# retir/Style-Big-GAN

Hardware: AMD Instinct MI355X
Metric: images/sec (G+D step) StyleGAN2-ADA 256x256 bf16 (higher is better)
Workload: dtype bf16; 1 GPU; configs/sg2ada.yaml @ 256x256: sg2_classic G (skip) + D (orig), softplus + R1(0.01)/4, idle Greg slot /16 (G lr x 16/17), global batch 64 = 1 rank(s) x 2 round(s) x batch_gpu 32 (the rounds of a phase evaluated in one pass, minibatch-std groups and loss those of the separate rounds), bf16 from 8x8 up (num_fp16_res 6; the reference recipe defaults to 4), conv_clamp 256, ADA off; global_batch=64, per_rank_batch=64, parallelism=dp1

## Files before the change

include/sbg_hip.h:

```cpp
#ifndef SBG_HIP_H
#define SBG_HIP_H

#include <stdint.h>

#ifdef __cplusplus
extern "C" {
#endif

typedef void* sbg_stream_t;

enum sbg_status {
    SBG_OK = 0,
    SBG_ERR_INVALID = 1,
    SBG_ERR_UNSUPPORTED = 2,
    SBG_ERR_LAUNCH = 3
};

enum sbg_dtype { SBG_F32 = 0, SBG_F16 = 1, SBG_BF16 = 2 };

enum sbg_act {
    SBG_ACT_LINEAR = 1, SBG_ACT_RELU = 2, SBG_ACT_LRELU = 3, SBG_ACT_TANH = 4, SBG_ACT_SIGMOID = 5,
    SBG_ACT_ELU = 6, SBG_ACT_SELU = 7, SBG_ACT_SOFTPLUS = 8, SBG_ACT_SWISH = 9
};

// ... 44 lines not shown
    int accumulate;
    const float* bias; const float* noise; int64_t noise_stride_n;
    int act; float alpha, gain, clamp;
    void* workspace; int ksplit;
    int nphase; int ph_ntaps[4], ph_oh[4], ph_ow[4]; int64_t ph_yoff[4];
} sbg_conv_params;
int64_t sbg_conv2d_igemm_workspace(const sbg_conv_params* p);
int     sbg_conv2d_igemm(const sbg_conv_params* p, sbg_stream_t stream);


typedef struct sbg_wgrad_params {
    const void* a; const void* b; float* out; void* workspace;
    int dtype;
    int N, PH, PW, Ca, BH, BW, Cb;
    int64_t as_n, as_h, as_w;
    int64_t bs_n, bs_h, bs_w;
    int stride;
    int ntaps;
    int tap_dy[SBG_MAX_TAPS], tap_dx[SBG_MAX_TAPS];
    int accumulate;
} sbg_wgrad_params;
int64_t sbg_conv2d_wgrad_workspace(const sbg_wgrad_params* p);
int     sbg_conv2d_wgrad(const sbg_wgrad_params* p, sbg_stream_t stream);


int sbg_scale_nc(const void* x, const float* a, const float* z, void* y, int dtype, int layout,
                 int N, int C, int64_t HW, int64_t z_stride_n, sbg_stream_t stream);
int sbg_scale_shift_nc(const void* x, const float* a, const float* b, void* y, int dtype, int layout,
                       int N, int C, int64_t HW, sbg_stream_t stream);

int sbg_dot_hw_splits(int layout, int N, int C, int64_t HW);
int sbg_dot_hw(const void* u, const void* v, float* partial, int dtype, int layout,
               int N, int C, int64_t HW, sbg_stream_t stream);
int sbg_moments_hw(const void* x, float* r, int dtype, int N, int C, int64_t HW, sbg_stream_t stream);

typedef struct sbg_gg_problem {
    const float *a0, *b0, *a1, *b1;
    float* c; const float* bias; float* rowsum;
    int64_t a0_rs, a0_cs, b0_rs, b0_cs, a1_rs, a1_cs, b1_rs, b1_cs, c_rs, c_cs;
    int M, N, K0, K1, nterms;
    float alpha0, alpha1, bias_scale, rowsum_scale;
} sbg_gg_problem;
int sbg_grouped_gemm(const sbg_gg_problem* problems, int count, sbg_stream_t stream);

int sbg_dot_hw_scale_supported(int C);
int sbg_dot_hw_scale(const void* u, const void* v, const float* scale, void* y, float* partial, int dtype,
// ... 129 lines not shown
```

style-big-gan_amd/_lib.py:

```python
import ctypes
import os
import threading

import torch

_HERE = os.path.dirname(os.path.abspath(__file__))
LIB_PATH = os.environ.get("SBG_HIP_LIBRARY") or os.path.join(_HERE, "libsbg_hip.so")

SBG_F32, SBG_F16, SBG_BF16 = 0, 1, 2
SBG_MAX_TAPS = 16

_DTYPES = {torch.float32: SBG_F32, torch.float16: SBG_F16, torch.bfloat16: SBG_BF16}


def dtype_code(dtype):
    try:
        return _DTYPES[dtype]
    except KeyError:
        raise RuntimeError(f"style_big_gan_amd: unsupported dtype {dtype} (float32 / float16 / bfloat16 only)")


class UpfirdnParams(ctypes.Structure):
    _fields_ = [
        ("x", ctypes.c_void_p), ("f", ctypes.c_void_p), ("y", ctypes.c_void_p),
# ... 81 lines not shown
QUANT_RULES = {"grid": 0, "clamp": 1}
RESAMPLE_VARIANTS = {0: "h", 1: "v"}
PR_VARIANTS = {0: "single", 1: "split", 2: "merge", 3: "norms"}
ATT_VARIANTS = {0: "single", 1: "stream", 2: "stream_stats", 3: "stream_dq", 4: "stream_dkv"}

_lib = None
_lock = threading.Lock()

_c = ctypes
SYMBOLS = [
    ("sbg_version", _c.c_int, []),
    ("sbg_last_error", _c.c_char_p, []),
    ("sbg_bias_act", _c.c_int, [_c.c_void_p] * 6 + [_c.c_int, _c.c_int, _c.c_int, _c.c_float, _c.c_float, _c.c_float,
                                                   _c.c_int64, _c.c_int, _c.c_int64, _c.c_void_p]),
    ("sbg_upfirdn2d_tail_supported", _c.c_int, [_c.POINTER(UpfirdnParams)]),
    ("sbg_upfirdn2d", _c.c_int, [_c.POINTER(UpfirdnParams), _c.c_void_p]),
    ("sbg_upfirdn2d_dact_rows", _c.c_int64, [_c.POINTER(UpfirdnParams)]),
    ("sbg_upfirdn2d_separable_supported", _c.c_int, [_c.c_int] * 3),
    ("sbg_upfirdn2d_separable", _c.c_int, [_c.c_void_p] * 3 + [_c.c_int] * 11 + [_c.c_float, _c.c_void_p]),
    ("sbg_conv2d_igemm_workspace", _c.c_int64, [_c.POINTER(ConvParams)]),
    ("sbg_conv2d_igemm", _c.c_int, [_c.POINTER(ConvParams), _c.c_void_p]),
    ("sbg_conv2d_wgrad_workspace", _c.c_int64, [_c.POINTER(WgradParams)]),
    ("sbg_conv2d_wgrad", _c.c_int, [_c.POINTER(WgradParams), _c.c_void_p]),
    ("sbg_scale_nc", _c.c_int, [_c.c_void_p] * 4 + [_c.c_int, _c.c_int, _c.c_int, _c.c_int, _c.c_int64, _c.c_int64, _c.c_void_p]),
    ("sbg_scale_shift_nc", _c.c_int, [_c.c_void_p] * 4 + [_c.c_int, _c.c_int, _c.c_int, _c.c_int, _c.c_int64, _c.c_void_p]),
    ("sbg_sn_workspace", _c.c_int64, [_c.c_int, _c.c_int]),
    ("sbg_sn_power_iteration", _c.c_int, [_c.c_void_p] * 6 + [_c.c_int, _c.c_int, _c.c_float, _c.c_void_p]),
    ("sbg_mbstd_workspace", _c.c_int64, [_c.c_int] * 5),
    ("sbg_mbstd_fwd", _c.c_int, [_c.c_void_p] * 3 + [_c.c_int] * 5 + [_c.c_void_p]),
    ("sbg_mbstd_bwd", _c.c_int, [_c.c_void_p] * 3 + [_c.c_int] * 5 + [_c.c_void_p]),
    ("sbg_split_bf16_cat", _c.c_int, [_c.c_void_p, _c.c_void_p, _c.c_int64, _c.c_int64, _c.c_int64, _c.c_int, _c.POINTER(_c.c_int), _c.c_void_p]),
    ("sbg_split_bf16_cat_nd", _c.c_int, [_c.c_void_p, _c.POINTER(_c.c_int64), _c.POINTER(_c.c_int64), _c.c_int, _c.c_void_p, _c.c_int, _c.POINTER(_c.c_int), _c.c_void_p]),
    ("sbg_attention_supported", _c.c_int, [_c.c_int] * 4),
    ("sbg_attention_fwd", _c.c_int, [_c.c_void_p] * 4 + [_c.c_int] * 5 + [_c.c_void_p]),
    ("sbg_attention_bwd_supported", _c.c_int, [_c.c_int] * 4),
    ("sbg_attention_bwd_workspace", _c.c_int64, [_c.c_int, _c.c_int]),
    ("sbg_attention_bwd", _c.c_int, [_c.c_void_p] * 8 + [_c.c_int] * 5 + [_c.c_void_p]),
    ("sbg_dot_hw_splits", _c.c_int, [_c.c_int, _c.c_int, _c.c_int, _c.c_int64]),
    ("sbg_dot_hw", _c.c_int, [_c.c_void_p] * 3 + [_c.c_int, _c.c_int, _c.c_int, _c.c_int, _c.c_int64, _c.c_void_p]),
    ("sbg_moments_hw", _c.c_int, [_c.c_void_p, _c.c_void_p, _c.c_int, _c.c_int, _c.c_int, _c.c_int64, _c.c_void_p]),
    ("sbg_grouped_gemm", _c.c_int, [_c.c_void_p, _c.c_int, _c.c_void_p]),
    ("sbg_dot_hw_scale_supported", _c.c_int, [_c.c_int]),
    ("sbg_dot_hw_scale", _c.c_int, [_c.c_void_p] * 5 + [_c.c_int, _c.c_int, _c.c_int, _c.c_int64, _c.c_void_p]),
    ("sbg_modconv_bwd_supported", _c.c_int, [_c.c_int]),
    ("sbg_modconv_bwd", _c.c_int, [_c.c_void_p] * 8 + [_c.c_int, _c.c_int, _c.c_int, _c.c_int64, _c.c_int64, _c.c_int, _c.c_float, _c.c_float, _c.c_float, _c.c_void_p]),
    ("sbg_modconv_bwd_prescaled", _c.c_int, [_c.c_void_p] * 10 + [_c.c_int, _c.c_int, _c.c_int, _c.c_int64, _c.c_int64, _c.c_int, _c.c_float, _c.c_float, _c.c_float, _c.c_void_p]),
# ... 111 lines not shown
```

style-big-gan_amd/csrc/conv_wgrad.hip:

```cpp
#include "conv_common.h"
#include "lds_asm.h"

namespace {

struct bf16_mfma {}; struct f16_mfma {};
template <class MF> struct Mfma;
template <> struct Mfma<bf16_mfma> {
    static __device__ __forceinline__ float4_t run(short8_t a, short8_t b, float4_t c) {
        return __builtin_amdgcn_mfma_f32_16x16x32_bf16(__builtin_bit_cast(bf16x8_t, a), __builtin_bit_cast(bf16x8_t, b), c, 0, 0, 0);
    }
};
template <> struct Mfma<f16_mfma> {
    static __device__ __forceinline__ float4_t run(short8_t a, short8_t b, float4_t c) {
        return __builtin_amdgcn_mfma_f32_16x16x32_f16(__builtin_bit_cast(f16x8_t, a), __builtin_bit_cast(f16x8_t, b), c, 0, 0, 0);
    }
};

struct WgradArgs {
    const unsigned short* a; const unsigned short* b; float* out; float* ws;
    int N, PH, PW, Ca, BH, BW, Cb;
    int64_t as_n, as_h, as_w, bs_n, bs_h, bs_w;
    int stride, ntaps;
    int tap_dy[SBG_MAX_TAPS], tap_dx[SBG_MAX_TAPS];
    int accumulate;
// ... 146 lines not shown
        float* slab = dst_base + (int64_t)(p.tap0 + t) * p.Ca * p.Cb;
#pragma unroll
        for (int i = 0; i < TA; i++)
#pragma unroll
            for (int j = 0; j < TB; j++) {
                const int cb = cb0 + wb + 16 * j + fi;
                if (cb >= p.Cb) continue;
#pragma unroll
                for (int e = 0; e < 4; e++) {
                    const int ca = ca0 + wa + 16 * i + 4 * fg + e;
                    if (ca >= p.Ca) continue;
                    float* d = slab + (int64_t)ca * p.Cb + cb;
                    const float v = acc[t][i][j][e];
                    *d = (direct && p.accumulate) ? *d + v : v;
                }
            }
    }
}



using sbgconv::lds_void_ptr;

template <class MF, int S, int BCA, int NSTAGE>
__global__ __launch_bounds__(512) void conv_wgrad_rows_kernel(WgradArgs p, unsigned a_bytes, unsigned b_bytes)
{
    static_assert(BCA == 64 || BCA == 128, "a tile of 64 or 128 channels");
    static_assert(NSTAGE >= 2 && NSTAGE <= 6, "2..6 stages (the wait ladder covers five chunks in flight)");
    constexpr int BCB = 64, NT = 9, DEPTH = NSTAGE - 1;
    constexpr int TA = BCA / 32;
    constexpr int APIECES = BCA / 16;
    constexpr int PCOLS = S * 31 + 3;
    constexpr int PPR = (PCOLS + 7) / 8;
    constexpr int PROW = PPR * 8;
    constexpr int NWAVE = 8;
    constexpr int NPIECE = ((APIECES + 3 * PPR + NWAVE - 1) / NWAVE) * NWAVE;
    constexpr int PIECES = NPIECE / NWAVE;
    constexpr int NREAL = APIECES + 3 * PPR;
    constexpr int A_BYTES = APIECES * 1024, STAGE = NREAL * 1024, DUMP = NSTAGE * STAGE;

    extern __shared__ __attribute__((aligned(16))) unsigned char smem[];
    const int tid = threadIdx.x, lane = tid & 63;
    const int wave = __builtin_amdgcn_readfirstlane(tid >> 6);
    int ta_, tb_, split;
    if (!wgrad_decode_block(p, ta_, tb_, split)) return;
    const int ca0 = ta_ * BCA, cb0 = tb_ * BCB;
    const int chunk_begin = split * p.chunks_per_split;
    int chunk_end = chunk_begin + p.chunks_per_split;
    if (chunk_end > p.nchunks) chunk_end = p.nchunks;
    const int nloc = chunk_end - chunk_begin;
    const int xblocks = p.PW >> 5;
    const int dy0 = p.tap_dy[0], dx0 = p.tap_dx[0];

    __amdgpu_buffer_rsrc_t ar = __builtin_amdgcn_make_buffer_rsrc((void*)p.a, 0, (int)a_bytes, 0x00020000);
    __amdgpu_buffer_rsrc_t br = __builtin_amdgcn_make_buffer_rsrc((void*)p.b, 0, (int)b_bytes, 0x00020000);

    const int drow = lane >> 3, dchunk = lane & 7;
    auto src_chunk = [&](int R) { return (((dchunk >> 1) ^ ((R >> 1) & 3)) << 1) | (dchunk & 1); };

    struct ChunkC { int py, n, px0; unsigned char* st; };
    auto chunk_coords = [&](int loc) -> ChunkC {
        const int c = chunk_begin + loc;
        const int xb = c % xblocks, rowid = c / xblocks;
        ChunkC r; r.py = rowid % p.PH; r.n = rowid / p.PH; r.px0 = xb << 5; r.st = smem + (loc % NSTAGE) * STAGE;
        return r;
    };
    auto issue_piece = [&](const ChunkC& cc, int i) {
        const int py = cc.py, n = cc.n, px0 = cc.px0;
        unsigned char* st = cc.st;
        {
            const int piece = wave + NWAVE * i;
            if (piece < APIECES) {
                const int R = (piece & 3) * 8 + drow;
                const int ch = ca0 + (piece >> 2) * 64 + src_chunk(R) * 8;
                const unsigned okm = 0u - (unsigned)(ch < p.Ca);
                const unsigned real = (unsigned)(n * (int)p.as_n + py * (int)p.as_h + (px0 + R) * (int)p.as_w + ch) * 2u;
                __builtin_amdgcn_raw_ptr_buffer_load_lds(ar, (lds_void_ptr)(st + piece * 1024), 16, (real & okm) | (SBG_OOB_OFFSET & ~okm), 0, 0, 0);
            } else {
                const int q = piece - APIECES;
                const int r = q / PPR, jb = q - r * PPR;
                const int R = r * PROW + jb * 8 + drow;
                constexpr int NEVEN = (PCOLS + 1) / 2, EVROWS = ((NEVEN + 7) / 8) * 8;
                const int pcol = (S == 1) ? jb * 8 + drow : (jb * 8 < EVROWS ? 2 * (jb * 8 + drow) : 2 * (jb * 8 - EVROWS + drow) + 1);
                const int by = S * py + dy0 + r, bx = S * px0 + dx0 + pcol;
                const int ch = cb0 + src_chunk(R) * 8;
                const unsigned okm = 0u - (unsigned)((q < 3 * PPR) & (pcol < PCOLS) & ((unsigned)by < (unsigned)p.BH) & ((unsigned)bx < (unsigned)p.BW) & (ch < p.Cb));
                const unsigned real = (unsigned)(n * (int)p.bs_n + by * (int)p.bs_h + bx * (int)p.bs_w + ch) * 2u;
                unsigned char* dst = (q < 3 * PPR) ? st + A_BYTES + q * 1024 : smem + DUMP;
                __builtin_amdgcn_raw_ptr_buffer_load_lds(br, (lds_void_ptr)dst, 16, (real & okm) | (SBG_OOB_OFFSET & ~okm), 0, 0, 0);
            }
        }
    };
    auto issue = [&](int loc) {
        const ChunkC cc = chunk_coords(loc);
#pragma unroll
        for (int i = 0; i < PIECES; i++) issue_piece(cc, i);
    };
    constexpr bool late = true;

    const int wa = (wave >> 2) * (BCA / 2), wb = (wave & 3) * 16;
    const int fi = lane & 15, fg = lane >> 4, fq = fi >> 2, fp = fi & 3;
    const unsigned lds_base = (unsigned)(uintptr_t)((lds_void_ptr)smem);
    float4_t acc[NT][TA];
#pragma unroll
    for (int t = 0; t < NT; t++)
#pragma unroll
        for (int i = 0; i < TA; i++) acc[t][i] = float4_t{0.f, 0.f, 0.f, 0.f};

    auto frag_off = [&](int Rrel, int col) {
        const int chunk = (col >> 3) + (fp >> 1);
        const int sw = (((chunk >> 1) ^ ((Rrel >> 1) & 3)) << 1) | (chunk & 1);
// ... 14 lines not shown
        short4_t lo = lds_tr_read(base + off), hi = lds_tr_read(base + off + hi_off);
        return short8_t{lo[0], lo[1], lo[2], lo[3], hi[0], hi[1], hi[2], hi[3]};
    };

#pragma unroll
    for (int s = 0; s < DEPTH; s++) if (s < nloc) issue(s);
    for (int s = 0; s < nloc; s++) {
        {
            const int later = nloc - 1 - s;
            if (DEPTH >= 2 && later >= DEPTH - 1) asm volatile("s_waitcnt vmcnt(%0)" :: "n"((DEPTH - 1) * PIECES) : "memory");
            else if (DEPTH >= 3 && later == DEPTH - 2) asm volatile("s_waitcnt vmcnt(%0)" :: "n"((DEPTH >= 3 ? DEPTH - 2 : 0) * PIECES) : "memory");
            else if (DEPTH >= 4 && later == DEPTH - 3) asm volatile("s_waitcnt vmcnt(%0)" :: "n"((DEPTH >= 4 ? DEPTH - 3 : 0) * PIECES) : "memory");
            else if (DEPTH >= 5 && later == DEPTH - 4) asm volatile("s_waitcnt vmcnt(%0)" :: "n"((DEPTH >= 5 ? DEPTH - 4 : 0) * PIECES) : "memory");
            else                                       asm volatile("s_waitcnt vmcnt(0)" ::: "memory");
        }
        __builtin_amdgcn_s_barrier();
        const bool more = s + DEPTH < nloc;
        ChunkC nxt = chunk_coords(more ? s + DEPTH : s);
        if (more && !late) {
#pragma unroll
            for (int i = 0; i < PIECES; i++) issue_piece(nxt, i);
        }
        const unsigned stage = lds_base + (unsigned)((s % NSTAGE) * STAGE);
        short4_t alo[TA], ahi[TA], blo[3], bhi[3];
        sbg_static_for<TA>([&](auto it) {
            constexpr int i = decltype(it)::value;
            lds_tr_issue<0>(alo[i], stage + (unsigned)offA[i]);
            lds_tr_issue<16 * 128>(ahi[i], stage + (unsigned)offA[i]);
        });
        unsigned pb[3];
#pragma unroll
        for (int d = 0; d < 3; d++) pb[d] = stage + (unsigned)offB[d];
        auto issue_b = [&](auto tt) {
            constexpr int t = decltype(tt)::value, dyi = t / 3, dxi = t % 3, OFF = A_BYTES + dyi * PROW * 128;
            lds_tr_issue<OFF>(blo[t % 3], pb[dxi]);
            lds_tr_issue<OFF + 16 * 128>(bhi[t % 3], pb[dxi]);
        };
        issue_b(std::integral_constant<int, 0>{});
        issue_b(std::integral_constant<int, 1>{});
        sbg_static_for<9>([&](auto tt) {
            constexpr int t = decltype(tt)::value;
            if constexpr (t + 2 < 9) issue_b(std::integral_constant<int, t + 2>{});
            lds_wait<(t + 2 < 9 ? 4 : t + 1 < 9 ? 2 : 0)>(blo[t % 3], bhi[t % 3]);
            const short8_t fb = short8_t{blo[t % 3][0], blo[t % 3][1], blo[t % 3][2], blo[t % 3][3], bhi[t % 3][0], bhi[t % 3][1], bhi[t % 3][2], bhi[t % 3][3]};
#pragma unroll
            for (int i = 0; i < TA; i++) {
                const short8_t fa_i = short8_t{alo[i][0], alo[i][1], alo[i][2], alo[i][3], ahi[i][0], ahi[i][1], ahi[i][2], ahi[i][3]};
                acc[t][i] = Mfma<MF>::run(fa_i, fb, acc[t][i]);
            }
            if (more && late) {
                sbg_static_for<PIECES>([&](auto pt) {
                    constexpr int i = decltype(pt)::value;
                    if constexpr (i * 9 / PIECES == t) issue_piece(nxt, i);
                });
            }
        });
    }

    const bool direct = (p.nsplit == 1);
    float* dst_base = direct ? p.out : p.ws + (int64_t)split * p.ntaps_total * p.Ca * p.Cb;
    const int cb = cb0 + wb + fi;
#pragma unroll
    for (int t = 0; t < NT; t++) {
        if (t >= p.ntaps || cb >= p.Cb) continue;
        float* slab = dst_base + (int64_t)(p.tap0 + t) * p.Ca * p.Cb;
#pragma unroll
        for (int i = 0; i < TA; i++)
#pragma unroll
            for (int e = 0; e < 4; e++) {
                const int ca = ca0 + wa + 16 * i + 4 * fg + e;
                if (ca >= p.Ca) continue;
                float* d = slab + (int64_t)ca * p.Cb + cb;
                const float v = acc[t][i][e];
                *d = (direct && p.accumulate) ? *d + v : v;
            }
    }
// ... 108 lines not shown
struct ThinPlan { bool ok; int dymin, dxmin, RY, PCOLS, wave_lds, nwg; };

static ThinPlan thin_plan(const sbg_wgrad_params* q)
{
    ThinPlan t; t.ok = false;
    if (q->Ca > 32 || q->Cb > 32 || q->Ca * q->Cb > 512 || q->ntaps > 9 || q->ntaps < 1 || q->stride < 1 || q->stride > 2 || q->N < 1) return t;
    int dy0 = q->tap_dy[0], dy1 = dy0, dx0 = q->tap_dx[0], dx1 = dx0;
    for (int i = 1; i < q->ntaps; i++) {
        if (q->tap_dy[i] < dy0) dy0 = q->tap_dy[i]; if (q->tap_dy[i] > dy1) dy1 = q->tap_dy[i];
        if (q->tap_dx[i] < dx0) dx0 = q->tap_dx[i]; if (q->tap_dx[i] > dx1) dx1 = q->tap_dx[i];
    }
    if (dy1 - dy0 > 2 || dx1 - dx0 > 2) return t;
    t.dymin = dy0; t.dxmin = dx0; t.RY = dy1 - dy0 + 1; t.PCOLS = q->stride * 31 + (dx1 - dx0) + 1;
    t.wave_lds = ((32 * q->Ca + t.RY * t.PCOLS * q->Cb) * 2 + 15) & ~15;
    const int64_t nchunks = (int64_t)q->N * q->PH * ((q->PW + 31) / 32);
    int64_t nwg = (nchunks + 15) / 16;
    if (nwg > 2048) nwg = 2048;
    if (nwg < 1) nwg = 1;
    t.nwg = (int)nwg;
    t.ok = nchunks < INT32_MAX;
    return t;
}

static void plan_split(WgradArgs& a, int bca, int bcb, int target)
{
    a.atiles = (a.Ca + bca - 1) / bca;
    a.btiles = (a.Cb + bcb - 1) / bcb;
    a.nchunks = (int)((a.P + 31) / 32);
    const int tiles = a.atiles * a.btiles;
    int want = (target + tiles - 1) / tiles;
    int maxsplit = a.nchunks / 8; if (maxsplit < 1) maxsplit = 1;
    if (want > maxsplit) want = maxsplit;
    if (want < 1) want = 1;
    a.chunks_per_split = (a.nchunks + want - 1) / want;
    a.nsplit = (a.nchunks + a.chunks_per_split - 1) / a.chunks_per_split;
}

static bool use_big_tile(int ntaps) { return ntaps == 1; }

static int rows_bca(const WgradArgs& a)
{
    return a.Ca >= 128 ? 128 : 64;
}

static constexpr int rows_nstage(int stride, int bca)
{
    if (bca == 128) return 4;
    return stride == 1 ? 4 : 2;
}

static bool rows_kernel_ok(const sbg_wgrad_params* q, const WgradArgs& a)
{
    if ((q->stride != 1 && q->stride != 2) || (q->PW % 32) != 0 || q->ntaps != 9) return false;
    for (int t = 0; t < 9; t++)
        if (q->tap_dy[t] != q->tap_dy[0] + t / 3 || q->tap_dx[t] != q->tap_dx[0] + t % 3) return false;
    if (q->as_n < 0 || q->as_h < 0 || q->as_w < 0 || q->bs_n < 0 || q->bs_h < 0 || q->bs_w < 0) return false;
    const int64_t ab = 2 * ((int64_t)(q->N - 1) * q->as_n + (int64_t)(q->PH - 1) * q->as_h + (int64_t)(q->PW - 1) * q->as_w + q->Ca);
    const int64_t bb = 2 * ((int64_t)(q->N - 1) * q->bs_n + (int64_t)(q->BH - 1) * q->bs_h + (int64_t)(q->BW - 1) * q->bs_w + q->Cb);
    return ab < (int64_t)SBG_OOB_OFFSET && bb < (int64_t)SBG_OOB_OFFSET && a.P > 0;
}

static int fill_args(const sbg_wgrad_params* q, WgradArgs& a)
{
    SBG_CHECK(q && q->a && q->b && q->out, "conv2d_wgrad: null pointer");
    SBG_CHECK(q->dtype == SBG_BF16 || q->dtype == SBG_F16, "conv2d_wgrad: a/b must be bf16 or f16 (fp32 inputs are split by the host)");
    SBG_CHECK(q->N >= 0 && q->PH >= 1 && q->PW >= 1 && q->BH >= 1 && q->BW >= 1, "conv2d_wgrad: bad sizes");
    SBG_CHECK(q->Ca >= 8 && q->Cb >= 8 && (q->Ca % 8) == 0 && (q->Cb % 8) == 0, "conv2d_wgrad: channel counts must be multiples of 8 (pad on the host)");
    SBG_CHECK(q->ntaps >= 1 && q->ntaps <= SBG_MAX_TAPS, "conv2d_wgrad: 1..%d taps", SBG_MAX_TAPS);
    SBG_CHECK(q->stride >= 1, "conv2d_wgrad: stride must be >= 1");
    SBG_CHECK(sbg_aligned16(q->a) && sbg_aligned16(q->b), "conv2d_wgrad: a and b must be 16-byte aligned");
    SBG_CHECK((q->as_n % 8) == 0 && (q->as_h % 8) == 0 && (q->as_w % 8) == 0 && (q->bs_n % 8) == 0 && (q->bs_h % 8) == 0 && (q->bs_w % 8) == 0,
              "conv2d_wgrad: pixel / row strides must be multiples of 8 elements");
    a.a = (const unsigned short*)q->a; a.b = (const unsigned short*)q->b; a.out = q->out; a.ws = (float*)q->workspace;
    a.N = q->N; a.PH = q->PH; a.PW = q->PW; a.Ca = q->Ca; a.BH = q->BH; a.BW = q->BW; a.Cb = q->Cb;
    a.as_n = q->as_n; a.as_h = q->as_h; a.as_w = q->as_w; a.bs_n = q->bs_n; a.bs_h = q->bs_h; a.bs_w = q->bs_w;
    a.stride = q->stride; a.ntaps = q->ntaps; a.accumulate = q->accumulate;
    for (int t = 0; t < SBG_MAX_TAPS; t++) { a.tap_dy[t] = q->tap_dy[t]; a.tap_dx[t] = q->tap_dx[t]; }
    a.P = (int64_t)q->N * q->PH * q->PW;
    a.tap0 = 0; a.ntaps_total = q->ntaps;
    if (use_big_tile(q->ntaps)) plan_split(a, 128, 128, 1024); else plan_split(a, 64, 64, 1024);
    if (rows_kernel_ok(q, a)) plan_split(a, rows_bca(a), 64, 512);
    const ThinPlan tp = thin_plan(q);
    if (tp.ok) { a.atiles = a.btiles = 1; a.nsplit = 4 * tp.nwg; a.chunks_per_split = 0; }
    return SBG_OK;
}

template <class MF, int BCA, int BCB, int NT>
static int launch_wgrad(const WgradArgs& a, hipStream_t stream)
{
    constexpr int lds = 32 * (BCA * 2 + 32) + NT * 32 * (BCB * 2 + 32);
    auto kern = conv_wgrad_kernel<MF, BCA, BCB, NT>;
    if (lds > 64 * 1024 && !SBG_RAISE_LDS_ONCE(kern, lds))
        return sbg_fail(SBG_ERR_LAUNCH, "conv2d_wgrad: cannot raise the dynamic LDS limit to %d bytes", lds);
    SbgProfScope prof(stream, SBG_K_CONV_WGRAD, 2.0 * (double)a.P * a.Ca * (double)a.Cb * a.ntaps,
                      2.0 * (double)a.P * a.Ca + 2.0 * (double)a.N * a.BH * a.BW * a.Cb + 4.0 * a.ntaps * (double)a.Ca * a.Cb * (a.nsplit > 1 ? a.nsplit : 1),
                      {(int)(a.P > INT32_MAX ? INT32_MAX : a.P), a.Ca, a.Cb, a.ntaps, a.stride, a.nsplit, BCA * 1000 + BCB});
    SBG_LAUNCH(kern, dim3(wgrad_grid(a)), dim3(256), lds, stream, a);
    SBG_HIP_LAUNCH_CHECK();
    return SBG_OK;
}

}

extern "C" int64_t sbg_conv2d_wgrad_workspace(const sbg_wgrad_params* q)
{
    WgradArgs a;
    if (fill_args(q, a) != SBG_OK) return -1;
    if (a.nsplit <= 1) return 0;
    return (int64_t)a.nsplit * a.ntaps_total * a.Ca * a.Cb * (int64_t)sizeof(float);
}

extern "C" int sbg_conv2d_wgrad(const sbg_wgrad_params* q, sbg_stream_t stream)
{
    WgradArgs a;
    int rc = fill_args(q, a);
    if (rc != SBG_OK) return rc;
    hipStream_t s = (hipStream_t)stream;
    const int64_t out_n = (int64_t)a.ntaps_total * a.Ca * a.Cb;
    if (a.P == 0) {
        if (!a.accumulate) { if (hipMemsetAsync(a.out, 0, out_n * sizeof(float), s) != hipSuccess) return sbg_fail(SBG_ERR_LAUNCH, "conv2d_wgrad: memset failed"); }
        return SBG_OK;
    }
    SBG_CHECK(a.nsplit == 1 || a.ws != nullptr, "conv2d_wgrad: workspace required (%d pixel splits)", a.nsplit);
    const bool bf = (q->dtype == SBG_BF16);
    const ThinPlan tp = thin_plan(q);
    if (tp.ok) {
        const int ta = (a.Ca + 15) / 16, tb = (a.Cb + 15) / 16;
        const int lds = 4 * tp.wave_lds;
        SbgProfScope prof(s, SBG_K_CONV_WGRAD, 2.0 * (double)a.P * a.Ca * (double)a.Cb * a.ntaps,
                          2.0 * (double)a.P * a.Ca + 2.0 * (double)a.N * a.BH * a.BW * a.Cb + 4.0 * a.ntaps * (double)a.Ca * a.Cb * a.nsplit,
                          {(int)(a.P > INT32_MAX ? INT32_MAX : a.P), a.Ca, a.Cb, a.ntaps, a.stride, a.nsplit, 3000000 + ta * 10 + tb});
#define SBG_THIN_LAUNCH(MFT, A_, B_) do { auto kern = conv_wgrad_thin_kernel<MFT, A_, B_>; \
        if (lds > 64 * 1024 && !SBG_RAISE_LDS_ONCE(kern, lds)) return sbg_fail(SBG_ERR_LAUNCH, "conv2d_wgrad: cannot raise the dynamic LDS limit to %d bytes", lds); \
        SBG_LAUNCH(kern, dim3((unsigned)tp.nwg), dim3(256), lds, s, a, tp.dymin, tp.dxmin, tp.RY, tp.PCOLS, tp.wave_lds); } while (0)
        if (bf) { if (ta == 1 && tb == 1) SBG_THIN_LAUNCH(bf16_mfma, 1, 1); else if (ta == 2 && tb == 1) SBG_THIN_LAUNCH(bf16_mfma, 2, 1);
                  else if (ta == 1) SBG_THIN_LAUNCH(bf16_mfma, 1, 2); else SBG_THIN_LAUNCH(bf16_mfma, 2, 2); }
        else    { if (ta == 1 && tb == 1) SBG_THIN_LAUNCH(f16_mfma, 1, 1); else if (ta == 2 && tb == 1) SBG_THIN_LAUNCH(f16_mfma, 2, 1);
                  else if (ta == 1) SBG_THIN_LAUNCH(f16_mfma, 1, 2); else SBG_THIN_LAUNCH(f16_mfma, 2, 2); }
#undef SBG_THIN_LAUNCH
        SBG_HIP_LAUNCH_CHECK();
    } else if (rows_kernel_ok(q, a)) {
        const unsigned ab = (unsigned)(2 * ((int64_t)(q->N - 1) * q->as_n + (int64_t)(q->PH - 1) * q->as_h + (int64_t)(q->PW - 1) * q->as_w + q->Ca));
        const unsigned bb = (unsigned)(2 * ((int64_t)(q->N - 1) * q->bs_n + (int64_t)(q->BH - 1) * q->bs_h + (int64_t)(q->BW - 1) * q->bs_w + q->Cb));
        const int bca = rows_bca(a);
        const int s_ = q->stride;
        auto stage_kib = [](int S, int BCA) { const int ppr = (S * 31 + 3 + 7) / 8; return BCA / 16 + 3 * ppr; };
        const int lds = (rows_nstage(s_, bca) * stage_kib(s_, bca) + 1) * 1024;
        SbgProfScope prof(s, SBG_K_CONV_WGRAD, 2.0 * (double)a.P * a.Ca * (double)a.Cb * a.ntaps,
                          2.0 * (double)a.P * a.Ca + 2.0 * (double)a.N * a.BH * a.BW * a.Cb + 4.0 * a.ntaps * (double)a.Ca * a.Cb * (a.nsplit > 1 ? a.nsplit : 1),
                          {(int)(a.P > INT32_MAX ? INT32_MAX : a.P), a.Ca, a.Cb, a.ntaps, a.stride, a.nsplit, 1000000 + bca * 1000 + 64});
        const dim3 grid(wgrad_grid(a));
#define SBG_ROWS_LAUNCH(MFT, SS, BB) do { auto kern = conv_wgrad_rows_kernel<MFT, SS, BB, rows_nstage(SS, BB)>; \
        if (lds > 64 * 1024 && !SBG_RAISE_LDS_ONCE(kern, lds)) return sbg_fail(SBG_ERR_LAUNCH, "conv2d_wgrad: cannot raise the dynamic LDS limit to %d bytes", lds); \
        SBG_LAUNCH(kern, grid, dim3(512), lds, s, a, ab, bb); } while (0)
        if (s_ == 1 && bca == 64)       { if (bf) SBG_ROWS_LAUNCH(bf16_mfma, 1, 64);  else SBG_ROWS_LAUNCH(f16_mfma, 1, 64); }
        else if (s_ == 1)               { if (bf) SBG_ROWS_LAUNCH(bf16_mfma, 1, 128); else SBG_ROWS_LAUNCH(f16_mfma, 1, 128); }
        else if (bca == 64)             { if (bf) SBG_ROWS_LAUNCH(bf16_mfma, 2, 64);  else SBG_ROWS_LAUNCH(f16_mfma, 2, 64); }
        else                            { if (bf) SBG_ROWS_LAUNCH(bf16_mfma, 2, 128); else SBG_ROWS_LAUNCH(f16_mfma, 2, 128); }
#undef SBG_ROWS_LAUNCH
        SBG_HIP_LAUNCH_CHECK();
    } else if (use_big_tile(a.ntaps)) {
        rc = bf ? launch_wgrad<bf16_mfma, 128, 128, 1>(a, s) : launch_wgrad<f16_mfma, 128, 128, 1>(a, s);
        if (rc != SBG_OK) return rc;
    } else {
        const int total = a.ntaps;
        for (int t0 = 0; t0 < total; t0 += 9) {
            WgradArgs g = a;
            g.tap0 = t0; g.ntaps = (total - t0 < 9) ? total - t0 : 9;
            for (int t = 0; t < g.ntaps; t++) { g.tap_dy[t] = a.tap_dy[t0 + t]; g.tap_dx[t] = a.tap_dx[t0 + t]; }
            rc = bf ? launch_wgrad<bf16_mfma, 64, 64, 9>(g, s) : launch_wgrad<f16_mfma, 64, 64, 9>(g, s);
            if (rc != SBG_OK) return rc;
        }
    }
    if (a.nsplit > 1) {
        SbgProfScope prof(s, SBG_K_WGRAD_REDUCE, 0.0, 4.0 * out_n * (a.nsplit + 1), {(int)out_n, a.nsplit});
        if (out_n >= (1 << 18) || a.nsplit < 16)
            SBG_LAUNCH(wgrad_reduce_kernel<1>, dim3(sbg_stream_grid(out_n, 256)), dim3(256), 0, s, a.ws, a.out, out_n, a.nsplit, a.accumulate);
        else if (out_n >= (1 << 14))
            SBG_LAUNCH(wgrad_reduce_kernel<4>, dim3(sbg_stream_grid(out_n * 4, 256)), dim3(256), 0, s, a.ws, a.out, out_n, a.nsplit, a.accumulate);
        else
            SBG_LAUNCH(wgrad_reduce_kernel<64>, dim3(sbg_stream_grid(out_n * 64, 256)), dim3(256), 0, s, a.ws, a.out, out_n, a.nsplit, a.accumulate);
// ... 5 lines not shown
```

style-big-gan_amd/torch_utils/ops/conv2d_gradfix.py:

```python
import contextlib

import weakref

import numpy as np

import torch

from ... import _lib

enabled = False
weight_gradients_disabled = False


@contextlib.contextmanager
def no_weight_gradients():
    global weight_gradients_disabled
    old = weight_gradients_disabled
    weight_gradients_disabled = True
    try:
        yield
    finally:
        weight_gradients_disabled = old


# ... 307 lines not shown
                    for j in range(kw) if (b + pw - j) % s == 0]
            if not taps:
                need_zero = True
                continue
            phases.append((a, b, goh, gow, taps))
    multi = len(passes) > 1 or any(len(t) > _lib.SBG_MAX_TAPS for *_, t in phases)
    y = torch.empty([n, cout, oh, ow], dtype=torch.float32 if multi else x.dtype, device=x.device, memory_format=torch.channels_last)
    if need_zero:
        y.zero_()
    first = True
    if (not multi and 2 <= len(phases) <= 4 and sum(len(t) for *_, t in phases) <= _lib.SBG_MAX_TAPS):
        xa, wa = passes[0]
        _igemm_phases(xa, wa.contiguous(), y, phases, s)
        return y
    for xa, wa in passes:
        wa = wa.contiguous()
        for a, b, goh, gow, taps in phases:
            for gi, grp in enumerate(_launch_groups(taps)):
                _igemm(xa, wa, y, grp, 1, goh, gow, y_off=(a, b), y_step=(s, s), accumulate=(not first) or gi > 0)
        first = False
    return y.to(x.dtype) if y.dtype != x.dtype else y


def _wgrad(a, b, stride, taps):
    lib = _lib.load()
    assert a.dtype == b.dtype and a.shape[0] == b.shape[0]
    ca, cb = a.shape[1], b.shape[1]
    pw = a.shape[3]
    if (len(taps) == 9 and stride in (1, 2) and pw in (8, 16)
            and all(taps[t] == (taps[0][0] + t // 3, taps[0][1] + t % 3) for t in range(9))):
        a = torch.nn.functional.pad(a, (0, 32 - pw))
    ap, bp = _pad_channels(a), _pad_channels(b)
    cap, cbp = ap.shape[1], bp.shape[1]
    out = torch.empty([len(taps), cap, cbp], dtype=torch.float32, device=a.device)
    first = True
    for aa, bb in _mfma_operands(ap, bp, 0, 0):
        aa, bb = _cl(aa), _cl(bb)
        for g0 in range(0, len(taps), _lib.SBG_MAX_TAPS):
            grp = taps[g0:g0 + _lib.SBG_MAX_TAPS]
            p = _lib.WgradParams()
            p.a, p.b, p.out = aa.data_ptr(), bb.data_ptr(), out[g0:].data_ptr()
            p.dtype = _lib.dtype_code(aa.dtype)
            p.N, p.PH, p.PW, p.Ca = aa.shape[0], aa.shape[2], aa.shape[3], cap
            p.BH, p.BW, p.Cb = bb.shape[2], bb.shape[3], cbp
            p.as_n, p.as_h, p.as_w = aa.stride(0), aa.stride(2), aa.stride(3)
            p.bs_n, p.bs_h, p.bs_w = bb.stride(0), bb.stride(2), bb.stride(3)
            p.stride, p.ntaps = stride, len(grp)
            for i, (dy, dx) in enumerate(grp):
                p.tap_dy[i], p.tap_dx[i] = dy, dx
            p.accumulate = int(not first)
            nbytes = lib.sbg_conv2d_wgrad_workspace(p)
            if nbytes < 0:
                _lib.check(1, "sbg_conv2d_wgrad_workspace")
            ws = torch.empty([max(nbytes, 4) // 4], dtype=torch.float32, device=a.device) if nbytes > 0 else None
            p.workspace = ws.data_ptr() if ws is not None else None
            _lib.check(lib.sbg_conv2d_wgrad(p, _lib.stream_ptr(a.device)), "sbg_conv2d_wgrad")
        first = False
    return out[:, :ca, :cb]



def _output_padding_for(transpose, stride, padding, in_hw, out_hw, k_hw):
    if transpose:
        return (0, 0)
    return tuple(in_hw[i] - (out_hw[i] - 1) * stride[i] - (1 - 2 * padding[i]) - (k_hw[i] - 1) for i in range(2))


class _Conv(torch.autograd.Function):

    @staticmethod
    def forward(ctx, x, w, cfg):
        transpose, stride, padding, output_padding = cfg[:4]
        wgain = cfg[4] if len(cfg) > 4 else 1.0
# ... 111 lines not shown
```

Baseline: 597.2 img/s.

## Process row pairs per chunk in stride-1 wgrad rows kernel to reuse B rows

Adds an R=2 variant of the rows-based weight-gradient kernel for stride-1, 32-wide inputs. Each chunk now loads two activation rows plus four gradient rows, and every loaded B fragment feeds the MFMAs of both A rows. Each B row used to be loaded for three separate chunks; now it is shared across the pair, cutting LDS staging and global traffic per output row. In exchange, each stage uses more LDS, the 64-channel case drops to two pipeline stages, there are half as many chunks for split-K parallelism, and the Python parameter setup is refactored into a helper.

```diff
diff --git a/include/sbg_hip.h b/include/sbg_hip.h
--- a/include/sbg_hip.h
+++ b/include/sbg_hip.h
@@ -90,6 +90,7 @@
 } sbg_wgrad_params;
 int64_t sbg_conv2d_wgrad_workspace(const sbg_wgrad_params* p);
 int     sbg_conv2d_wgrad(const sbg_wgrad_params* p, sbg_stream_t stream);
+int     sbg_conv2d_wgrad_rows_per_chunk(const sbg_wgrad_params* p);
 
 
 int sbg_scale_nc(const void* x, const float* a, const float* z, void* y, int dtype, int layout,
diff --git a/style-big-gan_amd/_lib.py b/style-big-gan_amd/_lib.py
--- a/style-big-gan_amd/_lib.py
+++ b/style-big-gan_amd/_lib.py
@@ -127,6 +127,7 @@
     ("sbg_conv2d_igemm", _c.c_int, [_c.POINTER(ConvParams), _c.c_void_p]),
     ("sbg_conv2d_wgrad_workspace", _c.c_int64, [_c.POINTER(WgradParams)]),
     ("sbg_conv2d_wgrad", _c.c_int, [_c.POINTER(WgradParams), _c.c_void_p]),
+    ("sbg_conv2d_wgrad_rows_per_chunk", _c.c_int, [_c.POINTER(WgradParams)]),
     ("sbg_scale_nc", _c.c_int, [_c.c_void_p] * 4 + [_c.c_int, _c.c_int, _c.c_int, _c.c_int, _c.c_int64, _c.c_int64, _c.c_void_p]),
     ("sbg_scale_shift_nc", _c.c_int, [_c.c_void_p] * 4 + [_c.c_int, _c.c_int, _c.c_int, _c.c_int, _c.c_int64, _c.c_void_p]),
     ("sbg_sn_workspace", _c.c_int64, [_c.c_int, _c.c_int]),
diff --git a/style-big-gan_amd/csrc/conv_wgrad.hip b/style-big-gan_amd/csrc/conv_wgrad.hip
--- a/style-big-gan_amd/csrc/conv_wgrad.hip
+++ b/style-big-gan_amd/csrc/conv_wgrad.hip
@@ -192,21 +192,24 @@
 
 using sbgconv::lds_void_ptr;
 
-template <class MF, int S, int BCA, int NSTAGE>
+template <class MF, int S, int BCA, int NSTAGE, int R>
 __global__ __launch_bounds__(512) void conv_wgrad_rows_kernel(WgradArgs p, unsigned a_bytes, unsigned b_bytes)
 {
     static_assert(BCA == 64 || BCA == 128, "a tile of 64 or 128 channels");
+    static_assert(R == 1 || R == 2, "one a row or a row pair per chunk");
     static_assert(NSTAGE >= 2 && NSTAGE <= 6, "2..6 stages (the wait ladder covers five chunks in flight)");
     constexpr int BCB = 64, NT = 9, DEPTH = NSTAGE - 1;
     constexpr int TA = BCA / 32;
-    constexpr int APIECES = BCA / 16;
+    constexpr int APT = BCA / 16;
+    constexpr int APIECES = R * APT;
+    constexpr int PR = S * (R - 1) + 3;
     constexpr int PCOLS = S * 31 + 3;
     constexpr int PPR = (PCOLS + 7) / 8;
     constexpr int PROW = PPR * 8;
     constexpr int NWAVE = 8;
-    constexpr int NPIECE = ((APIECES + 3 * PPR + NWAVE - 1) / NWAVE) * NWAVE;
+    constexpr int NPIECE = ((APIECES + PR * PPR + NWAVE - 1) / NWAVE) * NWAVE;
     constexpr int PIECES = NPIECE / NWAVE;
-    constexpr int NREAL = APIECES + 3 * PPR;
+    constexpr int NREAL = APIECES + PR * PPR;
     constexpr int A_BYTES = APIECES * 1024, STAGE = NREAL * 1024, DUMP = NSTAGE * STAGE;
 
     extern __shared__ __attribute__((aligned(16))) unsigned char smem[];
@@ -220,19 +223,20 @@
     if (chunk_end > p.nchunks) chunk_end = p.nchunks;
     const int nloc = chunk_end - chunk_begin;
     const int xblocks = p.PW >> 5;
+    const int prows = (p.PH + R - 1) / R;
     const int dy0 = p.tap_dy[0], dx0 = p.tap_dx[0];
 
     __amdgpu_buffer_rsrc_t ar = __builtin_amdgcn_make_buffer_rsrc((void*)p.a, 0, (int)a_bytes, 0x00020000);
     __amdgpu_buffer_rsrc_t br = __builtin_amdgcn_make_buffer_rsrc((void*)p.b, 0, (int)b_bytes, 0x00020000);
 
     const int drow = lane >> 3, dchunk = lane & 7;
-    auto src_chunk = [&](int R) { return (((dchunk >> 1) ^ ((R >> 1) & 3)) << 1) | (dchunk & 1); };
+    auto src_chunk = [&](int row) { return (((dchunk >> 1) ^ ((row >> 1) & 3)) << 1) | (dchunk & 1); };
 
     struct ChunkC { int py, n, px0; unsigned char* st; };
     auto chunk_coords = [&](int loc) -> ChunkC {
         const int c = chunk_begin + loc;
         const int xb = c % xblocks, rowid = c / xblocks;
-        ChunkC r; r.py = rowid % p.PH; r.n = rowid / p.PH; r.px0 = xb << 5; r.st = smem + (loc % NSTAGE) * STAGE;
+        ChunkC r; r.py = (rowid % prows) * R; r.n = rowid / prows; r.px0 = xb << 5; r.st = smem + (loc % NSTAGE) * STAGE;
         return r;
     };
     auto issue_piece = [&](const ChunkC& cc, int i) {
@@ -241,22 +245,23 @@
         {
             const int piece = wave + NWAVE * i;
             if (piece < APIECES) {
-                const int R = (piece & 3) * 8 + drow;
-                const int ch = ca0 + (piece >> 2) * 64 + src_chunk(R) * 8;
-                const unsigned okm = 0u - (unsigned)(ch < p.Ca);
-                const unsigned real = (unsigned)(n * (int)p.as_n + py * (int)p.as_h + (px0 + R) * (int)p.as_w + ch) * 2u;
+                const int arow = piece / APT, ap = piece % APT;
+                const int R_ = (ap & 3) * 8 + drow;
+                const int ch = ca0 + (ap >> 2) * 64 + src_chunk(R_) * 8;
+                const unsigned okm = 0u - (unsigned)((ch < p.Ca) & (py + arow < p.PH));
+                const unsigned real = (unsigned)(n * (int)p.as_n + (py + arow) * (int)p.as_h + (px0 + R_) * (int)p.as_w + ch) * 2u;
                 __builtin_amdgcn_raw_ptr_buffer_load_lds(ar, (lds_void_ptr)(st + piece * 1024), 16, (real & okm) | (SBG_OOB_OFFSET & ~okm), 0, 0, 0);
             } else {
                 const int q = piece - APIECES;
                 const int r = q / PPR, jb = q - r * PPR;
-                const int R = r * PROW + jb * 8 + drow;
+                const int R_ = r * PROW + jb * 8 + drow;
                 constexpr int NEVEN = (PCOLS + 1) / 2, EVROWS = ((NEVEN + 7) / 8) * 8;
                 const int pcol = (S == 1) ? jb * 8 + drow : (jb * 8 < EVROWS ? 2 * (jb * 8 + drow) : 2 * (jb * 8 - EVROWS + drow) + 1);
                 const int by = S * py + dy0 + r, bx = S * px0 + dx0 + pcol;
-                const int ch = cb0 + src_chunk(R) * 8;
-                const unsigned okm = 0u - (unsigned)((q < 3 * PPR) & (pcol < PCOLS) & ((unsigned)by < (unsigned)p.BH) & ((unsigned)bx < (unsigned)p.BW) & (ch < p.Cb));
+                const int ch = cb0 + src_chunk(R_) * 8;
+                const unsigned okm = 0u - (unsigned)((q < PR * PPR) & (pcol < PCOLS) & ((unsigned)by < (unsigned)p.BH) & ((unsigned)bx < (unsigned)p.BW) & (ch < p.Cb));
                 const unsigned real = (unsigned)(n * (int)p.bs_n + by * (int)p.bs_h + bx * (int)p.bs_w + ch) * 2u;
-                unsigned char* dst = (q < 3 * PPR) ? st + A_BYTES + q * 1024 : smem + DUMP;
+                unsigned char* dst = (q < PR * PPR) ? st + A_BYTES + q * 1024 : smem + DUMP;
                 __builtin_amdgcn_raw_ptr_buffer_load_lds(br, (lds_void_ptr)dst, 16, (real & okm) | (SBG_OOB_OFFSET & ~okm), 0, 0, 0);
             }
         }
@@ -317,36 +322,45 @@
             for (int i = 0; i < PIECES; i++) issue_piece(nxt, i);
         }
         const unsigned stage = lds_base + (unsigned)((s % NSTAGE) * STAGE);
-        short4_t alo[TA], ahi[TA], blo[3], bhi[3];
-        sbg_static_for<TA>([&](auto it) {
-            constexpr int i = decltype(it)::value;
-            lds_tr_issue<0>(alo[i], stage + (unsigned)offA[i]);
-            lds_tr_issue<16 * 128>(ahi[i], stage + (unsigned)offA[i]);
+        short4_t alo[R * TA], ahi[R * TA], blo[3], bhi[3];
+        sbg_static_for<R * TA>([&](auto it) {
+            constexpr int ar = decltype(it)::value / TA, i = decltype(it)::value % TA;
+            lds_tr_issue<ar * APT * 1024>(alo[ar * TA + i], stage + (unsigned)offA[i]);
+            lds_tr_issue<ar * APT * 1024 + 16 * 128>(ahi[ar * TA + i], stage + (unsigned)offA[i]);
         });
         unsigned pb[3];
 #pragma unroll
         for (int d = 0; d < 3; d++) pb[d] = stage + (unsigned)offB[d];
-        auto issue_b = [&](auto tt) {
-            constexpr int t = decltype(tt)::value, dyi = t / 3, dxi = t % 3, OFF = A_BYTES + dyi * PROW * 128;
-            lds_tr_issue<OFF>(blo[t % 3], pb[dxi]);
-            lds_tr_issue<OFF + 16 * 128>(bhi[t % 3], pb[dxi]);
+        constexpr int NF = 3 * PR;
+        static_assert(PIECES <= NF, "at most one DMA piece behind each fragment's MFMAs");
+        auto issue_b = [&](auto ff) {
+            constexpr int f = decltype(ff)::value, ri = f / 3, dxi = f % 3, OFF = A_BYTES + ri * PROW * 128;
+            lds_tr_issue<OFF>(blo[f % 3], pb[dxi]);
+            lds_tr_issue<OFF + 16 * 128>(bhi[f % 3], pb[dxi]);
         };
         issue_b(std::integral_constant<int, 0>{});
         issue_b(std::integral_constant<int, 1>{});
-        sbg_static_for<9>([&](auto tt) {
-            constexpr int t = decltype(tt)::value;
-            if constexpr (t + 2 < 9) issue_b(std::integral_constant<int, t + 2>{});
-            lds_wait<(t + 2 < 9 ? 4 : t + 1 < 9 ? 2 : 0)>(blo[t % 3], bhi[t % 3]);
-            const short8_t fb = short8_t{blo[t % 3][0], blo[t % 3][1], blo[t % 3][2], blo[t % 3][3], bhi[t % 3][0], bhi[t % 3][1], bhi[t % 3][2], bhi[t % 3][3]};
-#pragma unroll
-            for (int i = 0; i < TA; i++) {
-                const short8_t fa_i = short8_t{alo[i][0], alo[i][1], alo[i][2], alo[i][3], ahi[i][0], ahi[i][1], ahi[i][2], ahi[i][3]};
-                acc[t][i] = Mfma<MF>::run(fa_i, fb, acc[t][i]);
-            }
+        sbg_static_for<NF>([&](auto ff) {
+            constexpr int f = decltype(ff)::value;
+            if constexpr (f + 2 < NF) issue_b(std::integral_constant<int, f + 2>{});
+            lds_wait<(f + 2 < NF ? 4 : f + 1 < NF ? 2 : 0)>(blo[f % 3], bhi[f % 3]);
+            const short8_t fb = short8_t{blo[f % 3][0], blo[f % 3][1], blo[f % 3][2], blo[f % 3][3], bhi[f % 3][0], bhi[f % 3][1], bhi[f % 3][2], bhi[f % 3][3]};
+            sbg_static_for<R>([&](auto rr) {
+                constexpr int ar = decltype(rr)::value, dyi = f / 3 - S * ar;
+                if constexpr (dyi >= 0 && dyi < 3) {
+                    constexpr int t = 3 * dyi + f % 3;
+                    sbg_static_for<TA>([&](auto it) {
+                        constexpr int i = decltype(it)::value;
+                        const short4_t lo = alo[ar * TA + i], hi = ahi[ar * TA + i];
+                        const short8_t fa_i = short8_t{lo[0], lo[1], lo[2], lo[3], hi[0], hi[1], hi[2], hi[3]};
+                        acc[t][i] = Mfma<MF>::run(fa_i, fb, acc[t][i]);
+                    });
+                }
+            });
             if (more && late) {
                 sbg_static_for<PIECES>([&](auto pt) {
                     constexpr int i = decltype(pt)::value;
-                    if constexpr (i * 9 / PIECES == t) issue_piece(nxt, i);
+                    if constexpr (i * NF / PIECES == f) issue_piece(nxt, i);
                 });
             }
         });
@@ -501,7 +515,7 @@
     return t;
 }
 
-static void plan_split(WgradArgs& a, int bca, int bcb, int target)
+static void plan_split(WgradArgs& a, int bca, int bcb, int target, int rpc = 0)
 {
     a.atiles = (a.Ca + bca - 1) / bca;
     a.btiles = (a.Cb + bcb - 1) / bcb;
@@ -512,6 +526,10 @@
     if (want > maxsplit) want = maxsplit;
     if (want < 1) want = 1;
     a.chunks_per_split = (a.nchunks + want - 1) / want;
+    if (rpc == 2) {
+        a.nchunks = a.N * ((a.PH + 1) / 2);
+        a.chunks_per_split = (a.chunks_per_split + 1) / 2;
+    }
     a.nsplit = (a.nchunks + a.chunks_per_split - 1) / a.chunks_per_split;
 }
 
@@ -522,10 +540,16 @@
     return a.Ca >= 128 ? 128 : 64;
 }
 
-static constexpr int rows_nstage(int stride, int bca)
-{
+static constexpr int rows_nstage(int stride, int bca, int rpc)
+{
+    if (rpc == 2) return bca == 128 ? 4 : 2;
     if (bca == 128) return 4;
     return stride == 1 ? 4 : 2;
+}
+
+static constexpr int rows_rpc(int stride, int pw)
+{
+    return stride == 1 && pw == 32 ? 2 : 1;
 }
 
 static bool rows_kernel_ok(const sbg_wgrad_params* q, const WgradArgs& a)
@@ -537,6 +561,12 @@
     const int64_t ab = 2 * ((int64_t)(q->N - 1) * q->as_n + (int64_t)(q->PH - 1) * q->as_h + (int64_t)(q->PW - 1) * q->as_w + q->Ca);
     const int64_t bb = 2 * ((int64_t)(q->N - 1) * q->bs_n + (int64_t)(q->BH - 1) * q->bs_h + (int64_t)(q->BW - 1) * q->bs_w + q->Cb);
     return ab < (int64_t)SBG_OOB_OFFSET && bb < (int64_t)SBG_OOB_OFFSET && a.P > 0;
+}
+
+static int rows_path(const sbg_wgrad_params* q, const WgradArgs& a)
+{
+    if (a.P == 0 || thin_plan(q).ok || !rows_kernel_ok(q, a)) return 0;
+    return rows_rpc(q->stride, q->PW);
 }
 
 static int fill_args(const sbg_wgrad_params* q, WgradArgs& a)
@@ -558,7 +588,7 @@
     a.P = (int64_t)q->N * q->PH * q->PW;
     a.tap0 = 0; a.ntaps_total = q->ntaps;
     if (use_big_tile(q->ntaps)) plan_split(a, 128, 128, 1024); else plan_split(a, 64, 64, 1024);
-    if (rows_kernel_ok(q, a)) plan_split(a, rows_bca(a), 64, 512);
+    if (rows_kernel_ok(q, a)) plan_split(a, rows_bca(a), 64, 512, rows_rpc(q->stride, q->PW));
     const ThinPlan tp = thin_plan(q);
     if (tp.ok) { a.atiles = a.btiles = 1; a.nsplit = 4 * tp.nwg; a.chunks_per_split = 0; }
     return SBG_OK;
@@ -587,6 +617,12 @@
     if (fill_args(q, a) != SBG_OK) return -1;
     if (a.nsplit <= 1) return 0;
     return (int64_t)a.nsplit * a.ntaps_total * a.Ca * a.Cb * (int64_t)sizeof(float);
+}
+
+extern "C" int sbg_conv2d_wgrad_rows_per_chunk(const sbg_wgrad_params* q)
+{
+    WgradArgs a;
+    return fill_args(q, a) == SBG_OK ? rows_path(q, a) : 0;
 }
 
 extern "C" int sbg_conv2d_wgrad(const sbg_wgrad_params* q, sbg_stream_t stream)
@@ -618,24 +654,26 @@
                   else if (ta == 1) SBG_THIN_LAUNCH(f16_mfma, 1, 2); else SBG_THIN_LAUNCH(f16_mfma, 2, 2); }
 #undef SBG_THIN_LAUNCH
         SBG_HIP_LAUNCH_CHECK();
-    } else if (rows_kernel_ok(q, a)) {
+    } else if (const int rpc = rows_path(q, a)) {
         const unsigned ab = (unsigned)(2 * ((int64_t)(q->N - 1) * q->as_n + (int64_t)(q->PH - 1) * q->as_h + (int64_t)(q->PW - 1) * q->as_w + q->Ca));
         const unsigned bb = (unsigned)(2 * ((int64_t)(q->N - 1) * q->bs_n + (int64_t)(q->BH - 1) * q->bs_h + (int64_t)(q->BW - 1) * q->bs_w + q->Cb));
         const int bca = rows_bca(a);
         const int s_ = q->stride;
-        auto stage_kib = [](int S, int BCA) { const int ppr = (S * 31 + 3 + 7) / 8; return BCA / 16 + 3 * ppr; };
-        const int lds = (rows_nstage(s_, bca) * stage_kib(s_, bca) + 1) * 1024;
+        auto stage_kib = [](int S, int BCA, int R) { const int ppr = (S * 31 + 3 + 7) / 8; return R * (BCA / 16) + (S * (R - 1) + 3) * ppr; };
+        const int lds = (rows_nstage(s_, bca, rpc) * stage_kib(s_, bca, rpc) + 1) * 1024;
         SbgProfScope prof(s, SBG_K_CONV_WGRAD, 2.0 * (double)a.P * a.Ca * (double)a.Cb * a.ntaps,
                           2.0 * (double)a.P * a.Ca + 2.0 * (double)a.N * a.BH * a.BW * a.Cb + 4.0 * a.ntaps * (double)a.Ca * a.Cb * (a.nsplit > 1 ? a.nsplit : 1),
                           {(int)(a.P > INT32_MAX ? INT32_MAX : a.P), a.Ca, a.Cb, a.ntaps, a.stride, a.nsplit, 1000000 + bca * 1000 + 64});
         const dim3 grid(wgrad_grid(a));
-#define SBG_ROWS_LAUNCH(MFT, SS, BB) do { auto kern = conv_wgrad_rows_kernel<MFT, SS, BB, rows_nstage(SS, BB)>; \
+#define SBG_ROWS_LAUNCH(MFT, SS, BB, RR) do { auto kern = conv_wgrad_rows_kernel<MFT, SS, BB, rows_nstage(SS, BB, RR), RR>; \
         if (lds > 64 * 1024 && !SBG_RAISE_LDS_ONCE(kern, lds)) return sbg_fail(SBG_ERR_LAUNCH, "conv2d_wgrad: cannot raise the dynamic LDS limit to %d bytes", lds); \
         SBG_LAUNCH(kern, grid, dim3(512), lds, s, a, ab, bb); } while (0)
-        if (s_ == 1 && bca == 64)       { if (bf) SBG_ROWS_LAUNCH(bf16_mfma, 1, 64);  else SBG_ROWS_LAUNCH(f16_mfma, 1, 64); }
-        else if (s_ == 1)               { if (bf) SBG_ROWS_LAUNCH(bf16_mfma, 1, 128); else SBG_ROWS_LAUNCH(f16_mfma, 1, 128); }
-        else if (bca == 64)             { if (bf) SBG_ROWS_LAUNCH(bf16_mfma, 2, 64);  else SBG_ROWS_LAUNCH(f16_mfma, 2, 64); }
-        else                            { if (bf) SBG_ROWS_LAUNCH(bf16_mfma, 2, 128); else SBG_ROWS_LAUNCH(f16_mfma, 2, 128); }
+        if (rpc == 2 && bca == 64)      { if (bf) SBG_ROWS_LAUNCH(bf16_mfma, 1, 64, 2);  else SBG_ROWS_LAUNCH(f16_mfma, 1, 64, 2); }
+        else if (rpc == 2)              { if (bf) SBG_ROWS_LAUNCH(bf16_mfma, 1, 128, 2); else SBG_ROWS_LAUNCH(f16_mfma, 1, 128, 2); }
+        else if (s_ == 1 && bca == 64)  { if (bf) SBG_ROWS_LAUNCH(bf16_mfma, 1, 64, 1);  else SBG_ROWS_LAUNCH(f16_mfma, 1, 64, 1); }
+        else if (s_ == 1)               { if (bf) SBG_ROWS_LAUNCH(bf16_mfma, 1, 128, 1); else SBG_ROWS_LAUNCH(f16_mfma, 1, 128, 1); }
+        else if (bca == 64)             { if (bf) SBG_ROWS_LAUNCH(bf16_mfma, 2, 64, 1);  else SBG_ROWS_LAUNCH(f16_mfma, 2, 64, 1); }
+        else                            { if (bf) SBG_ROWS_LAUNCH(bf16_mfma, 2, 128, 1); else SBG_ROWS_LAUNCH(f16_mfma, 2, 128, 1); }
 #undef SBG_ROWS_LAUNCH
         SBG_HIP_LAUNCH_CHECK();
     } else if (use_big_tile(a.ntaps)) {
diff --git a/style-big-gan_amd/torch_utils/ops/conv2d_gradfix.py b/style-big-gan_amd/torch_utils/ops/conv2d_gradfix.py
--- a/style-big-gan_amd/torch_utils/ops/conv2d_gradfix.py
+++ b/style-big-gan_amd/torch_utils/ops/conv2d_gradfix.py
@@ -353,6 +353,21 @@
     return y.to(x.dtype) if y.dtype != x.dtype else y
 
 
+def _wgrad_params(aa, bb, out, stride, taps, accumulate=False):
+    p = _lib.WgradParams()
+    p.a, p.b, p.out = aa.data_ptr(), bb.data_ptr(), out.data_ptr()
+    p.dtype = _lib.dtype_code(aa.dtype)
+    p.N, p.PH, p.PW, p.Ca = aa.shape[0], aa.shape[2], aa.shape[3], aa.shape[1]
+    p.BH, p.BW, p.Cb = bb.shape[2], bb.shape[3], bb.shape[1]
+    p.as_n, p.as_h, p.as_w = aa.stride(0), aa.stride(2), aa.stride(3)
+    p.bs_n, p.bs_h, p.bs_w = bb.stride(0), bb.stride(2), bb.stride(3)
+    p.stride, p.ntaps = stride, len(taps)
+    for i, (dy, dx) in enumerate(taps):
+        p.tap_dy[i], p.tap_dx[i] = dy, dx
+    p.accumulate = int(accumulate)
+    return p
+
+
 def _wgrad(a, b, stride, taps):
     lib = _lib.load()
     assert a.dtype == b.dtype and a.shape[0] == b.shape[0]
@@ -368,18 +383,7 @@
     for aa, bb in _mfma_operands(ap, bp, 0, 0):
         aa, bb = _cl(aa), _cl(bb)
         for g0 in range(0, len(taps), _lib.SBG_MAX_TAPS):
-            grp = taps[g0:g0 + _lib.SBG_MAX_TAPS]
-            p = _lib.WgradParams()
-            p.a, p.b, p.out = aa.data_ptr(), bb.data_ptr(), out[g0:].data_ptr()
-            p.dtype = _lib.dtype_code(aa.dtype)
-            p.N, p.PH, p.PW, p.Ca = aa.shape[0], aa.shape[2], aa.shape[3], cap
-            p.BH, p.BW, p.Cb = bb.shape[2], bb.shape[3], cbp
-            p.as_n, p.as_h, p.as_w = aa.stride(0), aa.stride(2), aa.stride(3)
-            p.bs_n, p.bs_h, p.bs_w = bb.stride(0), bb.stride(2), bb.stride(3)
-            p.stride, p.ntaps = stride, len(grp)
-            for i, (dy, dx) in enumerate(grp):
-                p.tap_dy[i], p.tap_dx[i] = dy, dx
-            p.accumulate = int(not first)
+            p = _wgrad_params(aa, bb, out[g0:], stride, taps[g0:g0 + _lib.SBG_MAX_TAPS], accumulate=not first)
             nbytes = lib.sbg_conv2d_wgrad_workspace(p)
             if nbytes < 0:
                 _lib.check(1, "sbg_conv2d_wgrad_workspace")
```

Result: no change. 598.7 img/s, median of 4 (+0.3%).
